# winlaic/ZipVoice

Measured on AMD Instinct MI355X. Metric: generated mel-frames/s (whole job) + RTF, ZipVoice 123M N_steps=16 batch=32/GPU, higher is better.
Workload: dtype bf16; 1 GPU; C2: ZipVoice 123M, N_steps=16, batch=32/GPU x (3 s prompt + 10 s generated; T=1219 frames), CFG g=1.0 (64 decoder rows per GPU), t_shift=0.5; model=zipvoice (zipvoice_base.json, synthetic seeded weights), global_batch=32, seq_len=1219, parallelism=dp1

## Files before the change

### include/zipvoice_hip.h

```cpp
#ifndef ZIPVOICE_HIP_H
#define ZIPVOICE_HIP_H

#include <stdint.h>

#ifdef __cplusplus
extern "C" {
#endif

typedef struct zv_engine* zv_handle;

enum zv_variant { ZV_ZIPVOICE = 0, ZV_DISTILL = 1, ZV_DIALOG = 2, ZV_DIALOG_STEREO = 3 };
enum zv_precision { ZV_FP32 = 0, ZV_BF16 = 1, ZV_MIXED = 2, ZV_FP8 = 3 };

#define ZV_MAX_STACKS 8

typedef struct {
  int variant;
  int precision;
  int feat_dim;
  int num_stacks;
  int downsampling_factor[ZV_MAX_STACKS];
  int num_layers[ZV_MAX_STACKS];
  int cnn_module_kernel[ZV_MAX_STACKS];
  int fm_decoder_dim, fm_decoder_feedforward_dim, fm_decoder_num_heads;
// ... 7 lines not shown
const char* zv_last_error(void);
const char* zv_version(void);

zv_handle zv_create(const zv_config* cfg);
void zv_destroy(zv_handle h);

int zv_set_weight(zv_handle h, const char* name, const float* host_data, int64_t numel);
int zv_finalize(zv_handle h);
int zv_reserve(zv_handle h, int max_batch, int max_frames);
int64_t zv_device_bytes(zv_handle h);

int zv_profile(int enable);
int zv_profile_report(char* buf, int buflen);

int64_t zv_host_block_count(void);

int zv_attn_fallbacks(zv_handle h, int reset, int64_t* host_counts);

int zv_attn2_check(int kernel, int form, int B, int L, int H, int nv, const float* qkp, const float* P,
                   const uint8_t* key_pad, const float* v, const float* y, int force_exact, float* out,
                   int64_t* counts);

int zv_bench_gemm(int M, int N, int K, int variant, int iters, int out_mode, float* ms_out);

int zv_gemm_selftest(int M, int N, int K, int variant, int mode, float* maxdiff, float* maxref);

enum zv_linear_form {
  ZV_LIN_PLAIN = 0,
  ZV_LIN_PLAIN_F32 = 1,
  ZV_LIN_RESID = 2,
  ZV_LIN_RESID_BYP = 3,
  ZV_LIN_RESID_RV = 4,
  ZV_LIN_RESID_RV_COPY = 5,
  ZV_LIN_TRANS = 6,
  ZV_LIN_NA = 7,
  ZV_LIN_GLU = 8,
  ZV_LIN_GLU_DW = 9
};
typedef struct {
  int M, N, K, split, form, act;
  int rows_per_group;
  int rpb;
  int guard;
  const float* A; const float* W; const float* bias;
  const float* resid;
  const float* orig;
// ... 275 lines not shown
```

### zipvoice_amd/csrc/zv_checks.inc

```
#pragma once

namespace {

struct ChkDev {
  std::vector<void*> ptrs;
  void* raw(size_t bytes) {
    void* p = nullptr;
    ZV_CHECK(ZV_BLOCKING(hipMalloc(&p, bytes + 256)));
    ptrs.push_back(p);
    return p;
  }
  template <typename T> T* make(size_t n) { return reinterpret_cast<T*>(raw(n * sizeof(T))); }
  template <typename T> T* zero(size_t n) {
    T* d = make<T>(n);
    ZV_CHECK(ZV_BLOCKING(hipMemset(d, 0, n * sizeof(T))));
    return d;
  }
  template <typename T> T* up(const T* host, size_t n) {
    T* d = make<T>(n);
    ZV_CHECK(ZV_BLOCKING(hipMemcpy(d, host, n * sizeof(T), hipMemcpyHostToDevice)));
    return d;
  }
  template <typename T> void down(T* host, const T* dev, size_t n) {
    ZV_CHECK(ZV_BLOCKING(hipMemcpy(host, dev, n * sizeof(T), hipMemcpyDeviceToHost)));
// ... 92 lines not shown
  hipLaunchKernelGGL(zv_fill_rand_bf16, dim3(4096), dim3(256), 0, s, A, (long)M * Kp, 1u);
  hipLaunchKernelGGL(zv_fill_rand_bf16, dim3(4096), dim3(256), 0, s, W, (long)Np * Kp, 2u);
  GemmParams p{};
  p.M = M; p.N = N; p.K = K; p.nz2 = 1; p.Brows = (int)Np;
  p.Ah = A; p.lda = Kp; p.Bh = W; p.ldb = Kp;
  p.C = C; p.ldc = N; p.Ch = Ch; p.ldch = N; p.rows_per_group = 1; p.rpb = 1;
  if (out_mode == 2) p.resid = C;
  if (out_mode == 3) p.act = 1;
  if (out_mode == 4) { p.C = nullptr; p.Ch = nullptr; }
  if (out_mode == 7) {
    p.C = nullptr; p.bias = dev.zero<float>((size_t)N); p.act = 1;
  }
  if (out_mode == 5 || out_mode == 6) {
    float* extra = dev.zero<float>(2 * (size_t)N + (out_mode == 6 ? mn : 0));
    p.resid = C; p.bias = extra;
    if (out_mode == 6) { p.byp = extra + N; p.orig = extra + 2 * N; }
  }
  switch (variant) {
    case 0: *ms_out = bench_variant<0>(p, iters, persistent, s); break;
    case 72: *ms_out = bench_variant<3>(p, iters, persistent, s); break;
    default:
      *ms_out = out_mode == 5 ? bench_variant<1>(p, iters, persistent, s) : bench_variant<2>(p, iters, persistent, s);
  }
  ZV_API_END
}

int zv_gemm_selftest(int M, int N, int K, int variant, int mode, float* maxdiff, float* maxref) {
  ZV_API_BEGIN
  ZV_REQUIRE(variant == 70 || variant == 71 || variant == 72, "selftest: unknown variant");
  ZV_REQUIRE(variant == 72 || mode == 2, "selftest: residual-only variant");
  ZV_REQUIRE(variant != 72 || mode != 2, "selftest: variant 40 has no residual form");
  ChkDev dev;
  hipStream_t s = nullptr;
  const long Kp = round_up(K, 64), Np = round_up(N, 256);
  const size_t mn = (size_t)M * N;
  bf16* A = dev.make<bf16>((size_t)M * Kp);
  bf16* W = dev.make<bf16>((size_t)Np * Kp);
  float* outs[2] = {dev.make<float>(mn), dev.make<float>(mn)};
  float* R = dev.make<float>(mn);
  float* res = dev.make<float>(2);
  hipLaunchKernelGGL(zv_fill_rand_bf16, dim3(4096), dim3(256), 0, s, A, (long)M * Kp, 1u);
  hipLaunchKernelGGL(zv_fill_rand_bf16, dim3(4096), dim3(256), 0, s, W, (long)Np * Kp, 2u);
  hipLaunchKernelGGL(zv_fill_rand_bf16, dim3(4096), dim3(256), 0, s, reinterpret_cast<bf16*>(R),
                     (long)M * N * 2, 3u);
  if (Kp > K) {
    hipLaunchKernelGGL(zv_zero_kpad_kernel, dim3(1024), dim3(256), 0, s, A, (long)M, (int)Kp, K);
// ... 1080 lines not shown
```

### zipvoice_amd/csrc/zv_gemm.inc

```
#pragma once
#include "zv_common.h"
#include "zv_mx8.inc"

typedef __attribute__((address_space(3))) void lds_void_t;
typedef __attribute__((address_space(1))) const void gbl_void_t;

enum { EPI_STD = 0, EPI_TRANS = 1, EPI_NA = 2, EPI_GLU = 3, EPI_SPEC = 4, EPI_MAG = 5 };

struct GemmParams {
  int M, N, K, nz2;
  int Brows;
  const bf16* Ah; const bf16* Al; long lda, sA1, sA2;
  const bf16* Bh; const bf16* Bl; long ldb, sB1, sB2;
  const float* bias;
  int act;
  const float* colscale;
  int spec_im_off;
  float* C; long ldc, sC1, sC2;
  bf16* Ch; bf16* Cl; long ldch, sCh1, sCh2;
  const bf16* mulh; const bf16* mull; long ldmul, smul1, smul2;
  const float* resid;
  const float* rowvec; long rowvec_ld; int rows_per_group;
  const float* orig; const float* byp;
  bf16* Cth; bf16* Ctl; long ldct; int rpb; long sCt;
// ... 606 lines not shown
      }
      const bool ok = col_ok && m < p.M;
      const long o = (long)m * p.ldch + (nb / 32) * 16 + c8;
      bf16x8 h, l;
#pragma unroll
      for (int e = 0; e < 8; ++e) {
        h[e] = (bf16)v[e];
        l[e] = (bf16)(v[e] - (float)h[e]);
      }
      unsigned long long ha = ok ? (unsigned long long)(p.Ch + o) : (unsigned long long)(p.sink + 512 + lane * 4);
      asm volatile("" : "+v"(ha));
      *(GLOBAL bf16x8*)(ha) = h;
      if constexpr (NS == 2) {
        unsigned long long la = ok ? (unsigned long long)(p.Cl + o) : (unsigned long long)(p.sink + 1024 + lane * 4);
        asm volatile("" : "+v"(la));
        *(GLOBAL bf16x8*)(la) = l;
      }
    }
    __builtin_amdgcn_wave_barrier();
    __builtin_amdgcn_s_waitcnt(0xC07F);
  });
}

template <int TM, int TN, int NS>
__device__ __forceinline__ void gemm_epilogue_na_c(const GemmParams& p, f32x4 (&acc)[TM][TN],
                                                   int m0, int n0, int lane, float* scr) {
  constexpr int LDW = EpiScratch<TN>::LDW;
  static_assert(TN == 3, "one 48-column [s16 | x16 | y16] group per wave");
  const int nbc = min(n0, p.N - 48);
  const bool col_ok = n0 < p.N;
  const int cbase16 = (n0 / 48) * 16;
  const int yrow = lane >> 2, c4 = (lane & 3) * 4;
  const f32x4 by = *reinterpret_cast<const f32x4*>(p.bias + nbc + 32 + c4);
  const int ch = lane & 15, rg = lane >> 4;
  const float bs_ = p.bias[nbc + ch], bx = p.bias[nbc + 16 + ch];
  int bb = (m0 + rg * 4) / p.rpb, lf = (m0 + rg * 4) % p.rpb;
  static_for<TM>([&](auto I_) {
    constexpr int i = decltype(I_)::value;
#pragma unroll
    for (int j = 0; j < TN; ++j)
#pragma unroll
      for (int r = 0; r < 4; ++r) scr[((lane >> 4) * 4 + r) * LDW + j * 16 + (lane & 15)] = acc[i][j][r];
    __builtin_amdgcn_s_waitcnt(0xC07F);
    __builtin_amdgcn_wave_barrier();
    const int mrow0 = m0 + i * 16;
    {
      const int m = mrow0 + yrow;
      float v[4];
#pragma unroll
      for (int e = 0; e < 4; ++e) v[e] = scr[yrow * LDW + 32 + c4 + e] + by[e];
      bf16x4 h, l;
#pragma unroll
      for (int e = 0; e < 4; ++e) {
        h[e] = (bf16)v[e];
        l[e] = (bf16)(v[e] - (float)h[e]);
      }
      const bool ok = col_ok && m < p.M;
      const long o = (long)m * p.ldch + cbase16 + c4;
// ... 12 lines not shown
      const int row = rg * 4 + e, m = mrow0 + row;
      const float sv = scr[row * LDW + ch] + bs_;
      const float xv = scr[row * LDW + 16 + ch] + bx;
      const float v = __fmul_rn(xv, tanh_fast(sv));
      const bf16 h = (bf16)v;
      const bool ok = col_ok && m < p.M;
      const long o = b2 * p.sCt + (long)(cbase16 + ch) * p.ldct + l2;
      unsigned long long ha = ok ? (unsigned long long)(p.Cth + o) : (unsigned long long)(p.sink + 2048 + lane);
      asm volatile("" : "+v"(ha));
      *(GLOBAL bf16*)(ha) = h;
      if constexpr (NS == 2) {
        unsigned long long la = ok ? (unsigned long long)(p.Ctl + o) : (unsigned long long)(p.sink + 2560 + lane);
        asm volatile("" : "+v"(la));
        *(GLOBAL bf16*)(la) = (bf16)(v - (float)h);
      }
      if (e < 3) adv_pos(b2, l2, 1, p.rpb);
    }
    adv_pos(bb, lf, 16, p.rpb);
    __builtin_amdgcn_wave_barrier();
    __builtin_amdgcn_s_waitcnt(0xC07F);
  });
}

template <int TM, int TN, int NS>
__device__ __forceinline__ void gemm_epilogue_trans_c(const GemmParams& p, f32x4 (&acc)[TM][TN],
                                                      int m0, int n0, int lane, float* scr) {
  constexpr int WN = EpiScratch<TN>::W, LDW = EpiScratch<TN>::LDW;
  constexpr int Q = (16 * WN) / (64 * 4);
  static_assert(64 % WN == 0 && Q >= 1, "a lane's column is fixed across strips");
  const int col = lane % WN, rg0 = lane / WN;
  const int n = n0 + col;
  const bool col_ok = n < p.N;
  const float bn = p.bias ? p.bias[min(n, p.N - 1)] : 0.f;
  int bb[Q], lf[Q];
#pragma unroll
  for (int q = 0; q < Q; ++q) {
    const int m = m0 + (rg0 + q * (64 / WN)) * 4;
    bb[q] = m / p.rpb;
    lf[q] = m % p.rpb;
  }
  static_for<TM>([&](auto I_) {
    constexpr int i = decltype(I_)::value;
#pragma unroll
    for (int j = 0; j < TN; ++j)
#pragma unroll
      for (int r = 0; r < 4; ++r) scr[((lane >> 4) * 4 + r) * LDW + j * 16 + (lane & 15)] = acc[i][j][r];
    __builtin_amdgcn_s_waitcnt(0xC07F);
    __builtin_amdgcn_wave_barrier();
    const int mrow0 = m0 + i * 16;
#pragma unroll
    for (int q = 0; q < Q; ++q) {
// ... 8 lines not shown
        const long o = b2 * p.sCt + (long)n * p.ldct + l2;
        unsigned long long ha = ok ? (unsigned long long)(p.Cth + o) : (unsigned long long)(p.sink + 2048 + lane);
        asm volatile("" : "+v"(ha));
        *(GLOBAL bf16*)(ha) = h;
        if constexpr (NS == 2) {
          unsigned long long la = ok ? (unsigned long long)(p.Ctl + o) : (unsigned long long)(p.sink + 2560 + lane);
          asm volatile("" : "+v"(la));
          *(GLOBAL bf16*)(la) = (bf16)(v - (float)h);
        }
        if (e < 3) adv_pos(b2, l2, 1, p.rpb);
      }
      adv_pos(bb[q], lf[q], 16, p.rpb);
    }
    __builtin_amdgcn_wave_barrier();
    __builtin_amdgcn_s_waitcnt(0xC07F);
  });
}

#ifndef ZV_GEMM_PRELOAD
#define ZV_GEMM_PRELOAD 1
#endif
template <int BM, int BN, int WGM, int WGN, int SPLIT, int EPI, int STAGES = 2, int OCC = 2,
          int BK = GEMM_BK, int RP = 0, int CONV = 0, int ROLE = 0,
          int PRELOAD = ZV_GEMM_PRELOAD, int MXO = 0>
__global__ __launch_bounds__(64 * WGM * WGN, OCC) void zv_gemm_kernel(GemmParams p) {
  constexpr int NW = WGM * WGN;
  constexpr int WM = BM / WGM, WN = BN / WGN;
  constexpr int TM = WM / 16, TN = WN / 16;
  constexpr int NS = (SPLIT == 3) ? 2 : 1;
  constexpr int NSA = (SPLIT == 3) ? 2 : 1, NSB = (SPLIT == 3 || SPLIT == 2) ? 2 : 1;
  constexpr bool MX = SPLIT == 8;
  constexpr int EB = MX ? 1 : 2;
  static_assert(MX ? (BK == MX8_KSTEP && STAGES == 2 && !CONV && !RP)
                   : (BK == 64 || BK == 32), "K step depth");
  static_assert(MXO == 0 || (ROLE >= 1 && EPI == EPI_STD), "fp8 copy out: counted STD epilogues");
  constexpr int RB = BK * EB, CPRW = RB / 16, RPP = 1024 / RB;
  constexpr int A_BYTES = BM * BK * EB, B_BYTES = BN * BK * EB;
  constexpr int SA_P = MX ? (BM + 63) / 64 : 0, SB_P = MX ? (BN + 63) / 64 : 0;
  constexpr int SC_OFF = NS * (A_BYTES + B_BYTES);
  static_assert((SA_P + SB_P) % NW == 0, "MX scale pieces: the same count per wave");
  constexpr int STAGE = gemm_stage_bytes<BM, BN, SPLIT, BK>();
  constexpr bool SWZ = BK == 32 && NW * EpiScratch<TN>::BYTES > STAGE;
  constexpr int A_PIECES = A_BYTES / 1024, B_PIECES = B_BYTES / 1024;
  constexpr int PER_WAVE = NSA * ((A_PIECES + NW - 1) / NW) + NSB * ((B_PIECES + NW - 1) / NW) + (SA_P + SB_P) / NW;
  static_assert(STAGES == 2 || (A_PIECES % NW == 0 && B_PIECES % NW == 0),
                "multi-stage pipeline needs pieces divisible by the wave count");
  static_assert(BM % 8 == 0 && BN % 8 == 0 && WM % 16 == 0 && WN % 16 == 0, "tile");
  constexpr int SCR = SWZ ? 16 * 16 * TN * 4 : EpiScratch<TN>::BYTES;
  static_assert(NW * SCR <= STAGE, "epilogue scratch must fit one ring stage");
  auto swz = [](int row) -> int { return RB == 128 ? (row & 7) : ((120 >> (2 * ((row >> 2) & 3))) & 3); };

  extern __shared__ __attribute__((aligned(16))) unsigned char smem[];

  const int tid = threadIdx.x, lane = tid & 63;
  const int wave = __builtin_amdgcn_readfirstlane(tid >> 6);
  const int wm0 = (wave / WGN) * WM, wn0 = (wave % WGN) * WN;
  const int ntn = (p.N + BN - 1) / BN, ntm = (p.M + BM - 1) / BM;
  const int ntiles = ntn * ntm;
  const int G = gridDim.x, Q = G >> 3;
  const int bslot = (blockIdx.x & 7) * Q + (blockIdx.x >> 3);
  const int my_tiles = (bslot < ntiles) ? (ntiles - 1 - bslot) / G + 1 : 0;
  const int z1 = blockIdx.z / p.nz2, z2 = blockIdx.z % p.nz2;
  const long aoff = z1 * p.sA1 + z2 * p.sA2, boff = z1 * p.sB1 + z2 * p.sB2;
  const bf16* Ah = p.Ah + aoff;
  const bf16* Al = (SPLIT == 3) ? p.Al + aoff : nullptr;
  const bf16* Bh = p.Bh + boff;
  const bf16* Bl = (NSB == 2) ? p.Bl + boff : nullptr;
  const int nk = (p.K + BK - 1) / BK;
  const int total = my_tiles * nk;

  int ld_step = 0, ld_it = 0, ld_kt = 0;
  constexpr int APW = (A_PIECES + NW - 1) / NW, BPW = (B_PIECES + NW - 1) / NW;
  constexpr int SPW = MX ? (SA_P + SB_P) / NW : 1;
  unsigned offa[APW], offb[BPW], offs[SPW];
  const int prow = lane / CPRW, ppos = lane % CPRW;
  auto set_ld_tile = [&]() {
    const int tile = ld_it * G + bslot;
    const int ld_m0 = (tile / ntn) * BM, ld_n0 = (tile % ntn) * BN;
#pragma unroll
    for (int i = 0; i < APW; ++i) {
      const int row = (wave + i * NW) * RPP + prow;
      const int gm = min(ld_m0 + row, p.M - 1);
      offa[i] = (unsigned)((long)gm * p.lda * EB + (ppos ^ swz(row)) * 16);
    }
#pragma unroll
    for (int i = 0; i < BPW; ++i) {
      const int row = (wave + i * NW) * RPP + prow;
      const int gn = min(ld_n0 + row, p.Brows - 1);
      offb[i] = (unsigned)((long)gn * p.ldb * EB + (ppos ^ swz(row)) * 16);
    }
    if constexpr (MX) {
#pragma unroll
      for (int i = 0; i < SPW; ++i) {
        const int sp = wave + i * NW;
        offs[i] = sp < SA_P ? (unsigned)((long)min(ld_m0 + sp * 64 + lane, p.M - 1) * p.ldas)
                            : (unsigned)((long)min(ld_n0 + (sp - SA_P) * 64 + lane, p.Brows - 1) * p.ldbs);
      }
    }
  };
  auto issue_to = [&](unsigned char* base) {
    const int k0 = ld_kt * BK;
// ... 140 lines not shown
    }
  };

  int step = 0;
  for (int it = 0; it < my_tiles; ++it) {
    f32x4 acc[TM][TN];
#pragma unroll
    for (int i = 0; i < TM; ++i)
#pragma unroll
      for (int j = 0; j < TN; ++j) acc[i][j] = f32x4{0.f, 0.f, 0.f, 0.f};
    for (int kt = 0; kt < nk; ++kt, ++step) {
      {
        const int ahead = min(STAGES - 2, total - 1 - step);
        if (ahead <= 0) wait_vmcnt<0>();
        else if (ahead == 1) wait_vmcnt<PER_WAVE>();
        else if (ahead == 2) wait_vmcnt<2 * PER_WAVE>();
        else wait_vmcnt<3 * PER_WAVE>();
      }
      asm volatile("s_waitcnt lgkmcnt(0)" ::: "memory");
      __builtin_amdgcn_s_barrier();
      if (ld_step < total) issue();
      mma_step(smem + (step % STAGES) * STAGE, acc);
    }
    const int tile = it * G + bslot;
    const int m0 = (tile / ntn) * BM, n0 = (tile % ntn) * BN;
    __builtin_amdgcn_s_barrier();
    float* scr = reinterpret_cast<float*>(smem + ((step - 1) % STAGES) * STAGE + wave * SCR);
    if constexpr (ROLE >= 1 && EPI == EPI_STD && !RP && !SWZ)
      gemm_epilogue_res<TM, TN, NS, ROLE == 2, ROLE != 3, MXO, ROLE == 4 || ROLE == 5, ROLE == 5>(
          p, acc, m0 + wm0, n0 + wn0, lane, scr);
    else if constexpr (ROLE == 3 && EPI == EPI_GLU && !SWZ)
      gemm_epilogue_glu_c<TM, TN, NS>(p, acc, m0 + wm0, n0 + wn0, lane, scr);
    else if constexpr (ROLE == 3 && EPI == EPI_NA && !SWZ)
      gemm_epilogue_na_c<TM, TN, NS>(p, acc, m0 + wm0, n0 + wn0, lane, scr);
    else if constexpr (ROLE == 3 && EPI == EPI_TRANS && !SWZ)
      gemm_epilogue_trans_c<TM, TN, NS>(p, acc, m0 + wm0, n0 + wn0, lane, scr);
    else
      gemm_epilogue<TM, TN, EPI, SWZ, RP>(p, acc, m0 + wm0, n0 + wn0, z1, z2, lane, scr);
    __builtin_amdgcn_s_waitcnt(0x0F70);
  }
}

constexpr int ZV_MAX_DEVICES = 64;
static int zv_cur_device() {
  int dev = 0;
  ZV_CHECK(hipGetDevice(&dev));
  ZV_REQUIRE(dev >= 0 && dev < ZV_MAX_DEVICES, "device ordinal out of range");
  return dev;
}
static float* zv_epi_sink() {
  static float* sink[ZV_MAX_DEVICES] = {};
  const int d = zv_cur_device();
  if (!sink[d]) ZV_CHECK(ZV_BLOCKING(hipMalloc(&sink[d], 64 * 1024)));
  return sink[d];
}
static volatile unsigned* zv_dev_err_host() {
  static unsigned* const h = [] {
    unsigned* w = nullptr;
    ZV_CHECK(ZV_BLOCKING(hipHostMalloc((void**)&w, 64, hipHostMallocMapped | hipHostMallocPortable)));
// ... 68 lines not shown
    if (SPLIT == 3 && !pr.Cl) { pr.Cl = reinterpret_cast<bf16*>(pr.sink + 8192); pr.ldch = 0; }
  }
  return pr;
}

template <int SPLIT, int ROLE, int MXO>
static double gemm_alg_bytes(const GemmParams& p, int nz) {
  if constexpr (ROLE == 1 || ROLE == 2 || ROLE == 4 || ROLE == 5) {
    constexpr int NA = (SPLIT == 3) ? 2 : 1, NB = (SPLIT == 3 || SPLIT == 2) ? 2 : 1;
    constexpr bool MX = SPLIT == 8;
    const double mn = (double)p.M * p.N * nz;
    return (MX ? (1.0 + 1.0 / MX8_BLOCK) * ((double)p.M * p.K + (double)p.N * p.K)
               : 2.0 * (NA * (double)p.M * p.K + NB * (double)p.N * p.K)) * nz +
           mn * (4.0 * (p.resid != nullptr) + 4.0 * (p.C != nullptr) + 4.0 * (p.orig != nullptr) +
                 2.0 * (p.Ch != nullptr && MXO != 2) + 2.0 * (p.Cl != nullptr) +
                 (MXO ? 1.0 + 1.0 / MX8_BLOCK : 0.0));
  }
  return 0.0;
}

struct ZvLaunchRec { int BM, BN, SPLIT, EPI, ROLE, k256, grid, aux; };
static thread_local ZvLaunchRec g_zv_last_launch = {};

template <int BM, int BN, int WGM, int WGN, int SPLIT, int EPI, int STAGES = 2, int OCC = 2,
          int BK = GEMM_BK, int RP = 0, int CONV = 0, int ROLE = 0, int MXO = 0>
static void launch_gemm(const GemmParams& p, int nz, hipStream_t s, const char* tag,
                        bool persistent = true, int gridx = 0) {
  constexpr int NS = (SPLIT == 3) ? 2 : 1;
  constexpr bool MX = SPLIT == 8;
  constexpr size_t lds = (size_t)STAGES * gemm_stage_bytes<BM, BN, SPLIT, BK>();
  static_assert(lds <= 160 * 1024, "LDS budget");
  static unsigned long long attr = 0;
  if (!((attr >> zv_cur_device()) & 1)) {
    ZV_CHECK(hipFuncSetAttribute(
        (const void*)zv_gemm_kernel<BM, BN, WGM, WGN, SPLIT, EPI, STAGES, OCC, BK, RP, CONV, ROLE, ZV_GEMM_PRELOAD, MXO>,
        hipFuncAttributeMaxDynamicSharedMemorySize, (int)lds));
    attr |= 1ull << zv_cur_device();
  }
  ZV_REQUIRE(p.M > 0 && p.N > 0 && p.K > 0, "empty GEMM");
  if constexpr (MX)
    ZV_REQUIRE(p.As && p.Bs && p.K % MX8_KSTEP == 0 && p.lda % 16 == 0 && p.ldb % 16 == 0 &&
                   p.ldas * MX8_BLOCK >= p.K && p.ldbs * MX8_BLOCK >= p.K && nz == 1 && p.nz2 == 1,
               "MX-fp8 GEMM: scales present, K a multiple of 128, 16-B aligned rows");
  if constexpr (MXO > 0)
    ZV_REQUIRE(p.Cq && p.Cs && p.ldcq % MX8_KSTEP == 0 && p.N <= p.ldcq,
               "fp8 output copy: values and scales, row stride a multiple of 128");
  if constexpr (RP > 0)
    ZV_REQUIRE(p.residh && p.residl && p.Ch && p.Cl && !p.C && !p.resid && !p.orig && p.N % 8 == 0 &&
                   p.ldch % 8 == 0 && EPI == EPI_STD,
               "pair-residual GEMM: hi/lo residual in and out, N and ld multiples of 8");
  GemmParams pr = gemm_prep_epilogue<SPLIT, EPI, ROLE, MXO, RP>(p, nz);
  if constexpr (CONV)
    ZV_REQUIRE(p.conv_c > 0 && p.conv_c % BK == 0 && p.K % p.conv_c == 0 && p.lda == p.conv_c &&
                   p.conv_pad >= 0 && p.conv_d > 0 && p.nz2 == 1,
               "implicit-conv GEMM: channels a multiple of the K step, K = taps * channels");
  ZV_REQUIRE((long)p.M * p.lda * (MX ? 1 : 2) < (1L << 32) && (long)p.Brows * p.ldb * (MX ? 1 : 2) < (1L << 32),
             "GEMM operand larger than the 4 GiB DMA offset range");
  const int tiles = cdiv(p.N, BN) * cdiv(p.M, BM);
  constexpr int NWB = WGM * WGN;
  const int bpc = std::max(1, std::min({2, (int)((160 * 1024) / lds), std::max(1, OCC * 4 / NWB)}));
  static_assert(lds <= 160 * 1024, "LDS budget (ring + epilogue scratch)");
  if (gridx < 0) persistent = false;
  int G = (zv_num_cus() * (gridx > 0 ? gridx : bpc) + nz - 1) / nz;
  G = persistent ? std::min(G, tiles) : tiles;
  G = std::max(8, (G + 7) / 8 * 8);
  char dtag[160];
  if (g_zv_prof.detail) {
    snprintf(dtag, sizeof(dtag), "%s M=%d N=%d K=%d z=%d tile=%dx%d", tag, p.M, p.N, p.K, nz, BM, BN);
    tag = dtag;
  }
  g_zv_last_launch = ZvLaunchRec{BM, BN, SPLIT, EPI, ROLE, 0, G, STAGES * 16 + OCC};
  const double bytes = gemm_alg_bytes<SPLIT, ROLE, MXO>(p, nz);
  ZvProfScope prof(tag, 2.0 * p.M * p.N * (double)p.K * nz, bytes, s);
  hipLaunchKernelGGL((zv_gemm_kernel<BM, BN, WGM, WGN, SPLIT, EPI, STAGES, OCC, BK, RP, CONV, ROLE, ZV_GEMM_PRELOAD, MXO>), dim3(G, 1, nz),
                     dim3(64 * WGM * WGN), lds, s, pr);
  ZV_LAUNCH_CHECK();
}
```

### zipvoice_amd/csrc/zv_linear.inc

```
#pragma once
#include "zv_gemm.inc"
#include "zv_gemm256.inc"
#include "zv_weights.inc"

#ifndef ZV_WSPLIT_T_STAGES
#define ZV_WSPLIT_T_STAGES 3
#endif

namespace {

struct Act {
  bf16* h = nullptr;
  bf16* l = nullptr;
  long ld = 0;
  uint8_t* q = nullptr;
  uint8_t* qs = nullptr;
  long ldq = 0;
};

struct Out {
  float* C = nullptr; long ldc = 0;
  Act act;
  int act_fn = 0;
  const float* resid = nullptr;
  const float* rowvec = nullptr; long rowvec_ld = 0; int rows_per_group = 1;
  const float* orig = nullptr; const float* byp = nullptr;
  const bf16* residh = nullptr; const bf16* residl = nullptr;
  const bf16* origh = nullptr; const bf16* origl = nullptr;
};

template <int BM, int BN, int SPLIT, int EPI, int STAGES = 2, int OCC = 2, int ROLE = 0, int MXO = 0,
          int BK = GEMM_BK>
void gemm_tile(const GemmParams& p, hipStream_t s, const char* tag) {
  launch_gemm<BM, BN, 2, 2, SPLIT, EPI, STAGES, OCC, BK, 0, 0, ROLE, MXO>(p, 1, s, tag, true, -1);
}

struct LinearPolicy {
  int res_counted = 31;
  int gemm256 = 2;
  static constexpr int gemm256_min_tiles = 256;

  LinearPolicy() {
    auto envi = [](const char* k, int d) { const char* v = getenv(k); return v ? atoi(v) : d; };
    res_counted = envi("ZV_RES_COUNTED", 31);
    if (res_counted == 1) res_counted = 31;
    else if (res_counted >= 32) res_counted &= 31;
    gemm256 = envi("ZV_GEMM256", 2);
  }

  static long tiles128(const GemmParams& p) { return (long)cdiv(p.M, 128) * cdiv(p.N, 128); }
  static bool under_half_tile_per_cu(const GemmParams& p) { return tiles128(p) < zv_num_cus() / 2; }
  static bool under_3half_tiles_per_cu(const GemmParams& p) { return tiles128(p) < zv_num_cus() * 3 / 2; }
  bool use_gemm256(const GemmParams& p) const {
    return gemm256 != 0 && !p.Cl && !p.As && p.N % 8 == 0 && (p.act == 0 || p.act == 1) &&
           p.lda % 8 == 0 && p.ldb % 8 == 0 && p.lda >= round_up(p.K, GEMM_BK) &&
           p.ldb >= round_up(p.K, GEMM_BK) && p.Brows >= p.N &&
           (long)cdiv(p.M, 256) * cdiv(p.N, 256) >= gemm256_min_tiles;
  }

  static GemmParams gp_linear(const Linear& Lw, const Act& A, long M) {
    GemmParams p{};
    p.M = (int)M; p.N = Lw.N; p.K = Lw.K; p.nz2 = 1; p.Brows = Lw.Npad;
    p.Ah = A.h; p.Al = A.l; p.lda = A.ld;
    p.Bh = Lw.hi; p.Bl = Lw.lo; p.ldb = Lw.Kpad;
    p.bias = Lw.b; p.rows_per_group = 1; p.rpb = 1;
    return p;
  }
  static GemmParams gp_linear8(const Linear& Lw, const Act& A, long M) {
    GemmParams p = gp_linear(Lw, A, M);
    p.Ah = reinterpret_cast<const bf16*>(A.q); p.Al = nullptr; p.lda = A.ldq;
// ... 136 lines not shown
          return true;
        }
      launch_resid<SPLIT, 4>(p, s, tag);
    } else {
      launch_resid<SPLIT, 1>(p, s, split ? "gemm_fp32_resid" : "gemm_bf16_resid");
    }
    return false;
  }

  void attn_in_wsplit(const Linear& Lw, const Act& A, long M, const Out& o, hipStream_t s) {
    GemmParams p = gp_linear(Lw, A, M);
    p.Al = nullptr;
    p.Ch = o.act.h; p.Cl = nullptr; p.ldch = o.act.ld;
    ZV_REQUIRE(p.bias && p.Ch && !o.act.l && !o.C && !o.resid && !o.act_fn && Lw.lo && Lw.N % 8 == 0 &&
                   p.ldch % 8 == 0,
               "weight-split projection: bias -> 16-bit copy");
    gemm_tile<128, 64, 2, EPI_STD, 2, 2, 3>(p, s, "gemm_wsplit_n96");
  }

  template <int SPLIT>
  void launch_na_in(const GemmParams& p, hipStream_t s) {
    if constexpr (SPLIT == 1) {
      if ((res_counted & 4) && p.bias && p.N % 48 == 0 && p.ldch % 4 == 0)
        return gemm_tile<64, 96, 1, EPI_NA, 2, 3, 3>(p, s, "gemm_bf16_na");
    }
    gemm_tile<128, 96, SPLIT, EPI_NA>(p, s, SPLIT == 3 ? "gemm_fp32_na" : "gemm_bf16_na");
  }
  template <int SPLIT>
  void launch_value_t(const GemmParams& p, bool sa_split, bool has_lo, hipStream_t s) {
    const char* tag = SPLIT == 3 ? "gemm_fp32_t" : "gemm_bf16_t";
    if (sa_split) {
      ZV_REQUIRE(has_lo && (res_counted & 16), "weight-split value projection");
      gemm_tile<64, 64, 2, EPI_TRANS, ZV_WSPLIT_T_STAGES, ZV_WSPLIT_T_STAGES < 4 ? 2 : 1, 3>(p, s, "gemm_wsplit_t");
    } else if (res_counted & 16) {
      gemm_tile<64, 64, SPLIT, EPI_TRANS, 4, 2, 3>(p, s, tag);
    } else {
      gemm_tile<64, 64, SPLIT, EPI_TRANS>(p, s, tag);
    }
  }
  template <int SPLIT>
  void launch_glu_in(const GemmParams& p, bool g8, hipStream_t s) {
    if (g8) {
      ZV_REQUIRE(p.bias && p.N % 32 == 0 && p.ldch % 8 == 0, "fp8 GLU linear layout");
      return gemm_tile<128, 128, 8, EPI_GLU, 2, 2, 3, 0, MX8_KSTEP>(p, s, "gemm_fp8_glu");
    }
    const char* tag = SPLIT == 3 ? "gemm_fp32_glu" : "gemm_bf16_glu";
    if (!((res_counted & 8) && p.bias && p.N % 32 == 0 && p.ldch % 8 == 0))
      return gemm_tile<128, 128, SPLIT, EPI_GLU>(p, s, tag);
    if constexpr (SPLIT == 1) {
      if (use_gemm256(p)) return launch_gemm256<EPI_GLU, 3>(p, s, tag, gemm256 == 1);
      if (under_3half_tiles_per_cu(p)) return gemm_tile<64, 128, 1, EPI_GLU, 2, 3, 3>(p, s, tag);
    }
    gemm_tile<128, 128, SPLIT, EPI_GLU, 2, 2, 3>(p, s, tag);
  }
  bool glu_dw_fits(const GemmParams& p, int D, int ks) const {
    return (res_counted & 8) && D == 512 && p.N == 2 * D && (ks == 7 || ks == 15 || ks == 31) && p.bias &&
           !p.Cl && !p.As && p.lda % 8 == 0 && p.ldb % 8 == 0 && p.lda >= round_up(p.K, GEMM_BK) &&
           p.ldb >= round_up(p.K, GEMM_BK) && p.Brows >= p.N && p.ld_dw % 8 == 0;
// ... 10 lines not shown
```

### zipvoice_amd/engine.py

```python
from __future__ import annotations

import ctypes
import os
from typing import Dict, Optional

import numpy as np
import torch

from .config import ModelConfig
from .weights import check_state_dict

LIB_NAME = "libzipvoice_hip.so"
LIB_PATH = os.path.join(os.path.dirname(os.path.abspath(__file__)), LIB_NAME)
LIB_F16_PATH = os.path.join(os.path.dirname(os.path.abspath(__file__)), "libzipvoice_hip_f16.so")
MAX_STACKS = 8
VARIANT_ID = {"zipvoice": 0, "zipvoice_distill": 1, "zipvoice_dialog": 2,
              "zipvoice_dialog_stereo": 3}
PRECISION_ID = {"fp32": 0, "bf16": 1}
MODES = {"fp32": ("bf16", 0), "bf16": ("bf16", 1), "fp16": ("f16", 2),
         "fp16_plain": ("f16", 1), "bf16_mixed": ("bf16", 2), "fp8": ("bf16", 3)}


class ZvConfig(ctypes.Structure):
    _fields_ = [
# ... 112 lines not shown


class ZvNoiseCheckArgs(ctypes.Structure):
    _fields_ = [("mode", ctypes.c_int), ("where", ctypes.c_int),
                ("counter", ctypes.c_uint32 * 4), ("key", ctypes.c_uint32 * 2),
                ("count", ctypes.c_int64),
                ("words", ctypes.c_void_p), ("bits", ctypes.c_void_p), ("normals", ctypes.c_void_p)]


_P = ctypes.c_void_p
_I = ctypes.c_int
_F = ctypes.c_float
SIGNATURES = {
    "zv_last_error": (ctypes.c_char_p, []),
    "zv_version": (ctypes.c_char_p, []),
    "zv_create": (_P, [ctypes.POINTER(ZvConfig)]),
    "zv_destroy": (None, [_P]),
    "zv_set_weight": (_I, [_P, ctypes.c_char_p, _P, ctypes.c_int64]),
    "zv_finalize": (_I, [_P]),
    "zv_reserve": (_I, [_P, _I, _I]),
    "zv_device_bytes": (ctypes.c_int64, [_P]),
    "zv_profile": (_I, [_I]),
    "zv_bench_gemm": (_I, [_I, _I, _I, _I, _I, _I, ctypes.POINTER(ctypes.c_float)]),
    "zv_gemm_selftest": (_I, [_I, _I, _I, _I, _I, ctypes.POINTER(ctypes.c_float), ctypes.POINTER(ctypes.c_float)]),
    "zv_linear_check": (_I, [ctypes.POINTER(ZvLinearCheckArgs)]),
    "zv_ffn_check": (_I, [ctypes.POINTER(ZvFfnCheckArgs)]),
    "zv_dwconv_check": (_I, [ctypes.POINTER(ZvDwconvCheckArgs)]),
    "zv_stackedge_check": (_I, [ctypes.POINTER(ZvStackedgeCheckArgs)]),
    "zv_bigvgan_check": (_I, [ctypes.POINTER(ZvBigvganCheckArgs)]),
    "zv_solve_check": (_I, [ctypes.POINTER(ZvSolveCheckArgs)]),
    "zv_time_steps": (_I, [_F, _F, _I, _F, _P]),
    "zv_cfg_plan": (_I, [_F, _F, _I, _I, _I, _P, _P, _P, _P]),
    "zv_profile_report": (_I, [ctypes.c_char_p, _I]),
    "zv_host_block_count": (ctypes.c_int64, []),
    "zv_attn_fallbacks": (_I, [_P, _I, _P]),
    "zv_attn2_check": (_I, [_I, _I, _I, _I, _I, _I, _P, _P, _P, _P, _P, _I, _P, _P]),
    "zv_attn_plan": (_I, [_I, _I, _I, _I, _I, _P, _P, _P, _P]),
    "zv_mx8_quantize": (_I, [_P, _I, _I, _P, _P]),
    "zv_mx8_gemm_check": (_I, [_I, _I, _I, _P, _P, _P, _P, _P]),
    "zv_fm_decoder": (_I, [_P, _P, _P, _P, _P, _P, _P, _I, _I, _I, _P, _P]),
    "zv_velocity": (_I, [_P, _F, _F, _P, _P, _P, _P, _I, _I, _P, _P]),
    "zv_euler_sample": (_I, [_P, _P, _P, _P, _P, _I, _I, _I, _F, _F, _F, _F, _P]),
    "zv_velocity_rows": (_I, [_P, _F, _P, _P, _P, _P, _P, _I, _I, _P, _P]),
    "zv_euler_sample_rows": (_I, [_P, _P, _P, _P, _P, _I, _I, _I, _P, _F, _F, _F, _P]),
    "zv_euler_sample_sched": (_I, [_P, _P, _P, _P, _P, _I, _I, _P, _P]),
    "zv_sched_stats": (_I, [_P, _P]),
# ... 321 lines not shown
```

Measured before the change: 86510 mel-frames/s.

## Align GEMM M-tiles to utterance boundaries for vectorized transposed epilogue stores

Adds an utterance-aligned tile mapping (UTT) to the counted NA and transposed-value GEMM kernels, so each M-tile lies within one utterance. The transposed outputs are then packed across lanes with permlane16_swap and written as 16-byte vector stores along the time axis, replacing the scalar scatter through LDS scratch. It also adds a micro-benchmark entry point for these fused linears. In exchange, tiles at the end of each utterance can be partly empty when the utterance length is not a multiple of the tile height, which adds wasted work. The new path is on by default and can be switched off with an environment variable.

```diff
diff --git a/include/zipvoice_hip.h b/include/zipvoice_hip.h
--- a/include/zipvoice_hip.h
+++ b/include/zipvoice_hip.h
@@ -53,6 +53,8 @@
                    int64_t* counts);
 
 int zv_bench_gemm(int M, int N, int K, int variant, int iters, int out_mode, float* ms_out);
+
+int zv_bench_fused_linear(int form, int M, int N, int K, int rpb, int iters, float* ms_out);
 
 int zv_gemm_selftest(int M, int N, int K, int variant, int mode, float* maxdiff, float* maxref);
 
diff --git a/zipvoice_amd/csrc/zv_checks.inc b/zipvoice_amd/csrc/zv_checks.inc
--- a/zipvoice_amd/csrc/zv_checks.inc
+++ b/zipvoice_amd/csrc/zv_checks.inc
@@ -138,6 +138,43 @@
     default:
       *ms_out = out_mode == 5 ? bench_variant<1>(p, iters, persistent, s) : bench_variant<2>(p, iters, persistent, s);
   }
+  ZV_API_END
+}
+
+int zv_bench_fused_linear(int form, int M, int N, int K, int rpb, int iters, float* ms_out) {
+  ZV_API_BEGIN
+  ZV_REQUIRE((form == ZV_LIN_NA || form == ZV_LIN_TRANS) && M > 0 && N > 0 && K > 0 && rpb > 0 && iters > 0 &&
+                 ms_out && (form != ZV_LIN_NA || N % 48 == 0),
+             "zv_bench_fused_linear: form NA (N % 48 == 0) or TRANS, positive sizes");
+  ChkDev dev;
+  hipStream_t s = nullptr;
+  const long Kp = round_up(K, 64), Np = round_up(N, 128), Lpad = round_up(rpb, 64);
+  const int rows_t = form == ZV_LIN_NA ? N / 3 : N, nutt = cdiv(M, rpb);
+  bf16* A = dev.make<bf16>((size_t)M * Kp);
+  bf16* W = dev.make<bf16>((size_t)Np * Kp);
+  hipLaunchKernelGGL(zv_fill_rand_bf16, dim3(4096), dim3(256), 0, s, A, (long)M * Kp, 1u);
+  hipLaunchKernelGGL(zv_fill_rand_bf16, dim3(4096), dim3(256), 0, s, W, (long)Np * Kp, 2u);
+  GemmParams p{};
+  p.M = M; p.N = N; p.K = K; p.nz2 = 1; p.Brows = (int)Np;
+  p.Ah = A; p.lda = Kp; p.Bh = W; p.ldb = Kp;
+  p.bias = dev.zero<float>((size_t)N); p.rows_per_group = 1;
+  p.Cth = dev.zero<bf16>((size_t)nutt * rows_t * Lpad);
+  p.ldct = Lpad; p.rpb = rpb; p.sCt = (long)rows_t * Lpad;
+  if (form == ZV_LIN_NA) { p.ldch = round_up(rows_t, 8); p.Ch = dev.make<bf16>((size_t)M * p.ldch); }
+  LinearPolicy policy;
+  auto launch = [&]() {
+    if (form == ZV_LIN_NA) policy.launch_na_in<1>(p, s);
+    else policy.launch_value_t<1>(p, false, false, s);
+  };
+  ChkEvent e0, e1;
+  launch();
+  ZV_CHECK(hipEventRecord(e0.e, s));
+  for (int i = 0; i < iters; ++i) launch();
+  ZV_CHECK(hipEventRecord(e1.e, s));
+  ZV_CHECK(ZV_BLOCKING(hipEventSynchronize(e1.e)));
+  float ms = 0.f;
+  ZV_CHECK(hipEventElapsedTime(&ms, e0.e, e1.e));
+  *ms_out = ms / iters;
   ZV_API_END
 }
 
diff --git a/zipvoice_amd/csrc/zv_gemm.inc b/zipvoice_amd/csrc/zv_gemm.inc
--- a/zipvoice_amd/csrc/zv_gemm.inc
+++ b/zipvoice_amd/csrc/zv_gemm.inc
@@ -652,9 +652,73 @@
   });
 }
 
-template <int TM, int TN, int NS>
+__device__ __forceinline__ int utt_fofs(int lane) {
+  const int g = lane >> 4;
+  return ((g & 1) << 4) | ((g >> 1) << 3);
+}
+template <int NS>
+__device__ __forceinline__ void pack_trans4(const float (&v)[4], unsigned (&wh)[2], unsigned (&wl)[2]) {
+#pragma unroll
+  for (int r = 0; r < 2; ++r) {
+    const bf16x2 h = {(bf16)v[2 * r], (bf16)v[2 * r + 1]};
+    wh[r] = __builtin_bit_cast(unsigned, h);
+    if constexpr (NS == 2) {
+      const bf16x2 l = {(bf16)(v[2 * r] - (float)h[0]), (bf16)(v[2 * r + 1] - (float)h[1])};
+      wl[r] = __builtin_bit_cast(unsigned, l);
+    }
+  }
+}
+__device__ __forceinline__ unsigned mul_pack16(float x0, float t0, float x1, float t1) {
+#ifdef ZV_OPERAND_F16
+  unsigned w;
+  asm("v_fma_mixlo_f16 %0, %1, %2, 0\n\tv_fma_mixhi_f16 %0, %3, %4, 0\n\ts_nop 1"
+      : "=&v"(w) : "v"(x0), "v"(t0), "v"(x1), "v"(t1));
+  return w;
+#else
+  const bf16x2 h = {(bf16)__fmul_rn(x0, t0), (bf16)__fmul_rn(x1, t1)};
+  return __builtin_bit_cast(unsigned, h);
+#endif
+}
+template <int NS>
+__device__ __forceinline__ void store_trans8(const GemmParams& p, const unsigned (&wh)[2][2],
+                                             const unsigned (&wl)[2][2], long o, int nl, bool col_ok, int lane) {
+  typedef unsigned u32x4_t __attribute__((ext_vector_type(4)));
+  u32x4_t uh, ul;
+#pragma unroll
+  for (int r = 0; r < 2; ++r) {
+    const auto sw = __builtin_amdgcn_permlane16_swap(wh[0][r], wh[1][r], false, false);
+    uh[r] = sw[0];
+    uh[2 + r] = sw[1];
+    if constexpr (NS == 2) {
+      const auto sl = __builtin_amdgcn_permlane16_swap(wl[0][r], wl[1][r], false, false);
+      ul[r] = sl[0];
+      ul[2 + r] = sl[1];
+    }
+  }
+  const bool full = col_ok && nl >= 8;
+  unsigned long long ha = full ? (unsigned long long)(p.Cth + o) : (unsigned long long)(p.sink + 512 + lane * 4);
+  asm volatile("" : "+v"(ha));
+  *(GLOBAL u32x4_t*)(ha) = uh;
+  if constexpr (NS == 2) {
+    unsigned long long la = full ? (unsigned long long)(p.Ctl + o) : (unsigned long long)(p.sink + 1024 + lane * 4);
+    asm volatile("" : "+v"(la));
+    *(GLOBAL u32x4_t*)(la) = ul;
+  }
+  if (col_ok && nl > 0 && nl < 8) {
+    uint16_t* th = reinterpret_cast<uint16_t*>(p.Cth) + o;
+    uint16_t* tl = NS == 2 ? reinterpret_cast<uint16_t*>(p.Ctl) + o : nullptr;
+#pragma unroll
+    for (int e = 0; e < 7; ++e)
+      if (e < nl) {
+        th[e] = (uint16_t)(uh[e >> 1] >> (16 * (e & 1)));
+        if constexpr (NS == 2) tl[e] = (uint16_t)(ul[e >> 1] >> (16 * (e & 1)));
+      }
+  }
+}
+
+template <int TM, int TN, int NS, bool UTT = false>
 __device__ __forceinline__ void gemm_epilogue_na_c(const GemmParams& p, f32x4 (&acc)[TM][TN],
-                                                   int m0, int n0, int lane, float* scr) {
+                                                   int m0, int n0, int ub, int l0, int lane, float* scr) {
   constexpr int LDW = EpiScratch<TN>::LDW;
   static_assert(TN == 3, "one 48-column [s16 | x16 | y16] group per wave");
   const int nbc = min(n0, p.N - 48);
@@ -664,6 +728,49 @@
   const f32x4 by = *reinterpret_cast<const f32x4*>(p.bias + nbc + 32 + c4);
   const int ch = lane & 15, rg = lane >> 4;
   const float bs_ = p.bias[nbc + ch], bx = p.bias[nbc + 16 + ch];
+  if constexpr (UTT) {
+    static_assert(TM % 2 == 0, "aligned transposed stores pair the strips");
+    static_assert(NS == 1, "the counted NA epilogue runs the 16-bit product only (launch_na_in)");
+    const long orow = (long)ub * p.sCt + (long)(cbase16 + ch) * p.ldct;
+    static_for<TM / 2>([&](auto I_) {
+      constexpr int i = 2 * decltype(I_)::value;
+      unsigned wh[2][2], wl[2][2];
+#pragma unroll
+      for (int s = 0; s < 2; ++s) {
+        float xv[4], tv[4];
+#pragma unroll
+        for (int r = 0; r < 4; ++r) {
+          tv[r] = tanh_fast(acc[i + s][0][r] + bs_);
+          xv[r] = acc[i + s][1][r] + bx;
+        }
+        wh[s][0] = mul_pack16(xv[0], tv[0], xv[1], tv[1]);
+        wh[s][1] = mul_pack16(xv[2], tv[2], xv[3], tv[3]);
+      }
+      const int l = l0 + i * 16 + utt_fofs(lane);
+      store_trans8<NS>(p, wh, wl, orow + l, p.rpb - l, col_ok, lane);
+    });
+    static_for<TM>([&](auto I_) {
+      constexpr int i = decltype(I_)::value;
+#pragma unroll
+      for (int r = 0; r < 4; ++r) scr[(rg * 4 + r) * LDW + 32 + ch] = acc[i][2][r];
+      __builtin_amdgcn_s_waitcnt(0xC07F);
+      __builtin_amdgcn_wave_barrier();
+      float v[4];
+#pragma unroll
+      for (int e = 0; e < 4; ++e) v[e] = scr[yrow * LDW + 32 + c4 + e] + by[e];
+      bf16x4 h;
+#pragma unroll
+      for (int e = 0; e < 4; ++e) h[e] = (bf16)v[e];
+      const bool ok = col_ok && l0 + i * 16 + yrow < p.rpb;
+      const long o = (long)(m0 + i * 16 + yrow) * p.ldch + cbase16 + c4;
+      unsigned long long ha = ok ? (unsigned long long)(p.Ch + o) : (unsigned long long)(p.sink + 512 + lane * 4);
+      asm volatile("" : "+v"(ha));
+      *(GLOBAL bf16x4*)(ha) = h;
+      __builtin_amdgcn_wave_barrier();
+      __builtin_amdgcn_s_waitcnt(0xC07F);
+    });
+    return;
+  }
   int bb = (m0 + rg * 4) / p.rpb, lf = (m0 + rg * 4) % p.rpb;
   static_for<TM>([&](auto I_) {
     constexpr int i = decltype(I_)::value;
@@ -722,11 +829,36 @@
   });
 }
 
-template <int TM, int TN, int NS>
+template <int TM, int TN, int NS, bool UTT = false>
 __device__ __forceinline__ void gemm_epilogue_trans_c(const GemmParams& p, f32x4 (&acc)[TM][TN],
-                                                      int m0, int n0, int lane, float* scr) {
+                                                      int m0, int n0, int ub, int l0, int lane, float* scr) {
   constexpr int WN = EpiScratch<TN>::W, LDW = EpiScratch<TN>::LDW;
   constexpr int Q = (16 * WN) / (64 * 4);
+  if constexpr (UTT) {
+    static_assert(TM % 2 == 0, "aligned transposed stores pair the strips");
+    const int lf = l0 + utt_fofs(lane);
+    static_for<TN>([&](auto J_) {
+      constexpr int j = decltype(J_)::value;
+      const int n = n0 + j * 16 + (lane & 15);
+      const bool col_ok = n < p.N;
+      const float bn = p.bias ? p.bias[min(n, p.N - 1)] : 0.f;
+      const long orow = (long)ub * p.sCt + (long)n * p.ldct;
+      static_for<TM / 2>([&](auto I_) {
+        constexpr int i = 2 * decltype(I_)::value;
+        unsigned wh[2][2], wl[2][2];
+#pragma unroll
+        for (int s = 0; s < 2; ++s) {
+          float v[4];
+#pragma unroll
+          for (int r = 0; r < 4; ++r) v[r] = acc[i + s][j][r] + bn;
+          pack_trans4<NS>(v, wh[s], wl[s]);
+        }
+        const int l = lf + i * 16;
+        store_trans8<NS>(p, wh, wl, orow + l, p.rpb - l, col_ok, lane);
+      });
+    });
+    return;
+  }
   static_assert(64 % WN == 0 && Q >= 1, "a lane's column is fixed across strips");
   const int col = lane % WN, rg0 = lane / WN;
   const int n = n0 + col;
@@ -781,7 +913,7 @@
 #endif
 template <int BM, int BN, int WGM, int WGN, int SPLIT, int EPI, int STAGES = 2, int OCC = 2,
           int BK = GEMM_BK, int RP = 0, int CONV = 0, int ROLE = 0,
-          int PRELOAD = ZV_GEMM_PRELOAD, int MXO = 0>
+          int PRELOAD = ZV_GEMM_PRELOAD, int MXO = 0, int UTT = 0>
 __global__ __launch_bounds__(64 * WGM * WGN, OCC) void zv_gemm_kernel(GemmParams p) {
   constexpr int NW = WGM * WGN;
   constexpr int WM = BM / WGM, WN = BN / WGN;
@@ -814,8 +946,23 @@
   const int tid = threadIdx.x, lane = tid & 63;
   const int wave = __builtin_amdgcn_readfirstlane(tid >> 6);
   const int wm0 = (wave / WGN) * WM, wn0 = (wave % WGN) * WN;
-  const int ntn = (p.N + BN - 1) / BN, ntm = (p.M + BM - 1) / BM;
+  static_assert(!UTT || (ROLE == 3 && (EPI == EPI_NA || EPI == EPI_TRANS) && !SWZ),
+                "utterance-aligned tiles: the counted NA / transposed epilogues");
+  const int tpu = UTT ? (p.rpb + BM - 1) / BM : 1;
+  const int ntn = (p.N + BN - 1) / BN, ntm = UTT ? (p.M / p.rpb) * tpu : (p.M + BM - 1) / BM;
   const int ntiles = ntn * ntm;
+  auto tile_origin = [&](int tile, int& m0, int& n0, int& ub, int& l0) {
+    const int tm = tile / ntn;
+    n0 = (tile - tm * ntn) * BN;
+    if constexpr (UTT) {
+      ub = tm / tpu;
+      l0 = (tm - ub * tpu) * BM;
+      m0 = ub * p.rpb + l0;
+    } else {
+      ub = 0; l0 = 0;
+      m0 = tm * BM;
+    }
+  };
   const int G = gridDim.x, Q = G >> 3;
   const int bslot = (blockIdx.x & 7) * Q + (blockIdx.x >> 3);
   const int my_tiles = (bslot < ntiles) ? (ntiles - 1 - bslot) / G + 1 : 0;
@@ -834,8 +981,8 @@
   unsigned offa[APW], offb[BPW], offs[SPW];
   const int prow = lane / CPRW, ppos = lane % CPRW;
   auto set_ld_tile = [&]() {
-    const int tile = ld_it * G + bslot;
-    const int ld_m0 = (tile / ntn) * BM, ld_n0 = (tile % ntn) * BN;
+    int ld_m0, ld_n0, ld_ub, ld_l0;
+    tile_origin(ld_it * G + bslot, ld_m0, ld_n0, ld_ub, ld_l0);
 #pragma unroll
     for (int i = 0; i < APW; ++i) {
       const int row = (wave + i * NW) * RPP + prow;
@@ -1022,8 +1169,8 @@
       if (ld_step < total) issue();
       mma_step(smem + (step % STAGES) * STAGE, acc);
     }
-    const int tile = it * G + bslot;
-    const int m0 = (tile / ntn) * BM, n0 = (tile % ntn) * BN;
+    int m0, n0, ub, l0;
+    tile_origin(it * G + bslot, m0, n0, ub, l0);
     __builtin_amdgcn_s_barrier();
     float* scr = reinterpret_cast<float*>(smem + ((step - 1) % STAGES) * STAGE + wave * SCR);
     if constexpr (ROLE >= 1 && EPI == EPI_STD && !RP && !SWZ)
@@ -1032,9 +1179,9 @@
     else if constexpr (ROLE == 3 && EPI == EPI_GLU && !SWZ)
       gemm_epilogue_glu_c<TM, TN, NS>(p, acc, m0 + wm0, n0 + wn0, lane, scr);
     else if constexpr (ROLE == 3 && EPI == EPI_NA && !SWZ)
-      gemm_epilogue_na_c<TM, TN, NS>(p, acc, m0 + wm0, n0 + wn0, lane, scr);
+      gemm_epilogue_na_c<TM, TN, NS, UTT != 0>(p, acc, m0 + wm0, n0 + wn0, ub, l0 + wm0, lane, scr);
     else if constexpr (ROLE == 3 && EPI == EPI_TRANS && !SWZ)
-      gemm_epilogue_trans_c<TM, TN, NS>(p, acc, m0 + wm0, n0 + wn0, lane, scr);
+      gemm_epilogue_trans_c<TM, TN, NS, UTT != 0>(p, acc, m0 + wm0, n0 + wn0, ub, l0 + wm0, lane, scr);
     else
       gemm_epilogue<TM, TN, EPI, SWZ, RP>(p, acc, m0 + wm0, n0 + wn0, z1, z2, lane, scr);
     __builtin_amdgcn_s_waitcnt(0x0F70);
@@ -1149,8 +1296,13 @@
 struct ZvLaunchRec { int BM, BN, SPLIT, EPI, ROLE, k256, grid, aux; };
 static thread_local ZvLaunchRec g_zv_last_launch = {};
 
+static bool gemm_utt_ok(const GemmParams& p) {
+  return p.rpb > 0 && p.M % p.rpb == 0 && p.ldct >= p.rpb && p.ldct % 8 == 0 && p.sCt % 8 == 0 && p.Cth &&
+         (uintptr_t)p.Cth % 16 == 0 && (uintptr_t)p.Ctl % 16 == 0;
+}
+
 template <int BM, int BN, int WGM, int WGN, int SPLIT, int EPI, int STAGES = 2, int OCC = 2,
-          int BK = GEMM_BK, int RP = 0, int CONV = 0, int ROLE = 0, int MXO = 0>
+          int BK = GEMM_BK, int RP = 0, int CONV = 0, int ROLE = 0, int MXO = 0, int UTT = 0>
 static void launch_gemm(const GemmParams& p, int nz, hipStream_t s, const char* tag,
                         bool persistent = true, int gridx = 0) {
   constexpr int NS = (SPLIT == 3) ? 2 : 1;
@@ -1160,7 +1312,7 @@
   static unsigned long long attr = 0;
   if (!((attr >> zv_cur_device()) & 1)) {
     ZV_CHECK(hipFuncSetAttribute(
-        (const void*)zv_gemm_kernel<BM, BN, WGM, WGN, SPLIT, EPI, STAGES, OCC, BK, RP, CONV, ROLE, ZV_GEMM_PRELOAD, MXO>,
+        (const void*)zv_gemm_kernel<BM, BN, WGM, WGN, SPLIT, EPI, STAGES, OCC, BK, RP, CONV, ROLE, ZV_GEMM_PRELOAD, MXO, UTT>,
         hipFuncAttributeMaxDynamicSharedMemorySize, (int)lds));
     attr |= 1ull << zv_cur_device();
   }
@@ -1183,7 +1335,9 @@
                "implicit-conv GEMM: channels a multiple of the K step, K = taps * channels");
   ZV_REQUIRE((long)p.M * p.lda * (MX ? 1 : 2) < (1L << 32) && (long)p.Brows * p.ldb * (MX ? 1 : 2) < (1L << 32),
              "GEMM operand larger than the 4 GiB DMA offset range");
-  const int tiles = cdiv(p.N, BN) * cdiv(p.M, BM);
+  if constexpr (UTT)
+    ZV_REQUIRE(gemm_utt_ok(p), "utterance-aligned tiles: whole utterances, 16-B aligned V^T rows");
+  const int tiles = cdiv(p.N, BN) * (UTT ? (p.M / p.rpb) * cdiv(p.rpb, BM) : cdiv(p.M, BM));
   constexpr int NWB = WGM * WGN;
   const int bpc = std::max(1, std::min({2, (int)((160 * 1024) / lds), std::max(1, OCC * 4 / NWB)}));
   static_assert(lds <= 160 * 1024, "LDS budget (ring + epilogue scratch)");
@@ -1196,10 +1350,10 @@
     snprintf(dtag, sizeof(dtag), "%s M=%d N=%d K=%d z=%d tile=%dx%d", tag, p.M, p.N, p.K, nz, BM, BN);
     tag = dtag;
   }
-  g_zv_last_launch = ZvLaunchRec{BM, BN, SPLIT, EPI, ROLE, 0, G, STAGES * 16 + OCC};
+  g_zv_last_launch = ZvLaunchRec{BM, BN, SPLIT, EPI, ROLE, 0, G, STAGES * 16 + OCC + 256 * UTT};
   const double bytes = gemm_alg_bytes<SPLIT, ROLE, MXO>(p, nz);
   ZvProfScope prof(tag, 2.0 * p.M * p.N * (double)p.K * nz, bytes, s);
-  hipLaunchKernelGGL((zv_gemm_kernel<BM, BN, WGM, WGN, SPLIT, EPI, STAGES, OCC, BK, RP, CONV, ROLE, ZV_GEMM_PRELOAD, MXO>), dim3(G, 1, nz),
+  hipLaunchKernelGGL((zv_gemm_kernel<BM, BN, WGM, WGN, SPLIT, EPI, STAGES, OCC, BK, RP, CONV, ROLE, ZV_GEMM_PRELOAD, MXO, UTT>), dim3(G, 1, nz),
                      dim3(64 * WGM * WGN), lds, s, pr);
   ZV_LAUNCH_CHECK();
 }
diff --git a/zipvoice_amd/csrc/zv_linear.inc b/zipvoice_amd/csrc/zv_linear.inc
--- a/zipvoice_amd/csrc/zv_linear.inc
+++ b/zipvoice_amd/csrc/zv_linear.inc
@@ -30,15 +30,21 @@
 };
 
 template <int BM, int BN, int SPLIT, int EPI, int STAGES = 2, int OCC = 2, int ROLE = 0, int MXO = 0,
-          int BK = GEMM_BK>
+          int BK = GEMM_BK, int UTT = 0>
 void gemm_tile(const GemmParams& p, hipStream_t s, const char* tag) {
-  launch_gemm<BM, BN, 2, 2, SPLIT, EPI, STAGES, OCC, BK, 0, 0, ROLE, MXO>(p, 1, s, tag, true, -1);
+  launch_gemm<BM, BN, 2, 2, SPLIT, EPI, STAGES, OCC, BK, 0, 0, ROLE, MXO, UTT>(p, 1, s, tag, true, -1);
+}
+template <int BM, int BN, int SPLIT, int EPI, int STAGES, int OCC>
+void gemm_tile_t(const GemmParams& p, bool utt, hipStream_t s, const char* tag) {
+  if (utt) gemm_tile<BM, BN, SPLIT, EPI, STAGES, OCC, 3, 0, GEMM_BK, 1>(p, s, tag);
+  else gemm_tile<BM, BN, SPLIT, EPI, STAGES, OCC, 3>(p, s, tag);
 }
 
 struct LinearPolicy {
   int res_counted = 31;
   int gemm256 = 2;
   static constexpr int gemm256_min_tiles = 256;
+  bool utt_na = true, utt_t = true;
 
   LinearPolicy() {
     auto envi = [](const char* k, int d) { const char* v = getenv(k); return v ? atoi(v) : d; };
@@ -46,6 +52,9 @@
     if (res_counted == 1) res_counted = 31;
     else if (res_counted >= 32) res_counted &= 31;
     gemm256 = envi("ZV_GEMM256", 2);
+    const int ta = envi("ZV_TRANS_ALIGNED", 1);
+    utt_na = ta == 1 || ta == 2;
+    utt_t = ta == 1 || ta == 3;
   }
 
   static long tiles128(const GemmParams& p) { return (long)cdiv(p.M, 128) * cdiv(p.N, 128); }
@@ -228,18 +237,19 @@
   void launch_na_in(const GemmParams& p, hipStream_t s) {
     if constexpr (SPLIT == 1) {
       if ((res_counted & 4) && p.bias && p.N % 48 == 0 && p.ldch % 4 == 0)
-        return gemm_tile<64, 96, 1, EPI_NA, 2, 3, 3>(p, s, "gemm_bf16_na");
+        return gemm_tile_t<64, 96, 1, EPI_NA, 2, 3>(p, utt_na && gemm_utt_ok(p), s, "gemm_bf16_na");
     }
     gemm_tile<128, 96, SPLIT, EPI_NA>(p, s, SPLIT == 3 ? "gemm_fp32_na" : "gemm_bf16_na");
   }
   template <int SPLIT>
   void launch_value_t(const GemmParams& p, bool sa_split, bool has_lo, hipStream_t s) {
     const char* tag = SPLIT == 3 ? "gemm_fp32_t" : "gemm_bf16_t";
+    const bool utt = utt_t && gemm_utt_ok(p);
     if (sa_split) {
       ZV_REQUIRE(has_lo && (res_counted & 16), "weight-split value projection");
-      gemm_tile<64, 64, 2, EPI_TRANS, ZV_WSPLIT_T_STAGES, ZV_WSPLIT_T_STAGES < 4 ? 2 : 1, 3>(p, s, "gemm_wsplit_t");
+      gemm_tile_t<64, 64, 2, EPI_TRANS, ZV_WSPLIT_T_STAGES, ZV_WSPLIT_T_STAGES < 4 ? 2 : 1>(p, utt, s, "gemm_wsplit_t");
     } else if (res_counted & 16) {
-      gemm_tile<64, 64, SPLIT, EPI_TRANS, 4, 2, 3>(p, s, tag);
+      gemm_tile_t<64, 64, SPLIT, EPI_TRANS, 4, 2>(p, utt, s, tag);
     } else {
       gemm_tile<64, 64, SPLIT, EPI_TRANS>(p, s, tag);
     }
diff --git a/zipvoice_amd/engine.py b/zipvoice_amd/engine.py
--- a/zipvoice_amd/engine.py
+++ b/zipvoice_amd/engine.py
@@ -158,6 +158,7 @@
     "zv_device_bytes": (ctypes.c_int64, [_P]),
     "zv_profile": (_I, [_I]),
     "zv_bench_gemm": (_I, [_I, _I, _I, _I, _I, _I, ctypes.POINTER(ctypes.c_float)]),
+    "zv_bench_fused_linear": (_I, [_I, _I, _I, _I, _I, _I, ctypes.POINTER(ctypes.c_float)]),
     "zv_gemm_selftest": (_I, [_I, _I, _I, _I, _I, ctypes.POINTER(ctypes.c_float), ctypes.POINTER(ctypes.c_float)]),
     "zv_linear_check": (_I, [ctypes.POINTER(ZvLinearCheckArgs)]),
     "zv_ffn_check": (_I, [ctypes.POINTER(ZvFfnCheckArgs)]),
```

New measurement: 88100 mel-frames/s, median of 6. 1.02x the previous value.
